# cvg/glue-factory

Measured on AMD Instinct MI355X. Metric: image-pairs/sec (train step) SP+LightGlue N=2048 d=256 L=9, higher is better.
Workload: dtype bf16; 1 GPU; configs[1]: SuperPoint + LightGlue train step -- frozen SuperPoint-open forward on 2x32 synthetic 1024x1024 images resident in HBM (view1 = view0 warped by a sampled homography, SURVEY 8(d)(P); first block and the 64-channel 3x3 blocks as fused HIP kernels, library convolutions + fused HIP tails for the 128/256-channel blocks), homography ground truth (gf_gt_nn), LightGlue fwd + loss + bwd + fused; pairs_per_gpu=32, global_batch=32, keypoints=2048, descriptor_dim=256, layers=9, parallelism=dp1

## Files before the change

glue-factory_amd/csrc/attention.hip:

```cpp
#include "gf_launch.h"
#include "attn_common.h"

using namespace gfattn;

namespace {

bool bad_stride(const int64_t* s, int align) { return s[0] % align || s[1] % align || s[2] % align; }

int attn_params(AttnParams& p, const void* q, const void* k, const void* v, const void* o, const float* lse,
                int B, int H, int Nq, int Nk, int D, const int64_t* qs, const int64_t* ks, const int64_t* vs, const int64_t* os,
                float scale, int dtype, int flags, int known, bool o_f32_if_split) {
    if (D != 64 && D != 32 && D != 128) return GF_ERR_UNSUPPORTED;
    if (flags & ~known) return GF_ERR_UNSUPPORTED;
    if (D != 64 && (flags & GF_ATTN_SPLIT) && dtype != GF_F32) return GF_ERR_UNSUPPORTED;
    if (dtype == GF_F32) flags &= ~GF_ATTN_SPLIT;
    if ((flags & GF_ATTN_SPLIT) && !(kvdma_ok(Nk, ks[1]) && kvdma_ok(Nk, vs[1]))) return GF_ERR_UNSUPPORTED;
    if (B <= 0 || H <= 0 || Nq <= 0 || Nk <= 0) return GF_ERR_SHAPE;
    const int align = gf_vec_elems(dtype);
    if (bad_stride(qs, align) || bad_stride(ks, align) || bad_stride(vs, align) ||
        bad_stride(os, (o_f32_if_split && (flags & GF_ATTN_SPLIT)) ? 4 : align))
        return GF_ERR_ALIGN;
    p = {};
    p.q = q; p.k = k; p.v = v; p.o = const_cast<void*>(o); p.lse = const_cast<float*>(lse);
    p.B = B; p.H = H; p.Nq = Nq; p.Nk = Nk; p.scale = scale;
    host_split_scale(scale, p.p2, p.rr);
    p.flags = flags;
    p.sqb = qs[0]; p.sqn = qs[1]; p.sqh = qs[2];
    p.skb = ks[0]; p.skn = ks[1]; p.skh = ks[2];
    p.svb = vs[0]; p.svn = vs[1]; p.svh = vs[2];
    p.sob = os[0]; p.son = os[1]; p.soh = os[2];
    return 0;
}

bool lds_dma(const AttnParams& p, int dtype, int D) {
    return dtype == GF_BF16 && D == 64 && kvdma_ok(p.Nk, p.skn) && kvdma_ok(p.Nk, p.svn);
}
int launch_fwd(const AttnParams& p, hipStream_t st, int dtype, int D) {
    return lds_dma(p, dtype, D) ? launch_fwd3_bf16(p, st) : launch_fwd_generic(p, st, dtype, D);
}
int launch_bwd(const AttnParams& p, hipStream_t st, int dtype, int D) {
    if (dtype != GF_BF16 || D != 64) return launch_bwd_generic(p, st, dtype, D);
    if (int e = lds_dma(p, dtype, D) ? launch_dq3_bf16(p, st) : launch_dq_generic(p, st, dtype, D)) return e;
    return launch_dkv_bf16(p, st);
}

}

extern "C" int gf_attn_fwd(const void* q, const void* k, const void* v, void* o, float* lse,
                           int B, int H, int Nq, int Nk, int D,
                           const int64_t* q_strides, const int64_t* k_strides,
                           const int64_t* v_strides, const int64_t* o_strides,
                           float scale, int dtype, void* stream) {
    return gf_attn_fwd_ex(q, k, v, o, lse, B, H, Nq, Nk, D, q_strides, k_strides, v_strides, o_strides, scale, dtype, 0, nullptr, stream);
}
extern "C" int gf_attn_fwd_ex(const void* q, const void* k, const void* v, void* o, float* lse,
                              int B, int H, int Nq, int Nk, int D,
                              const int64_t* q_strides, const int64_t* k_strides,
                              const int64_t* v_strides, const int64_t* o_strides,
                              float scale, int dtype, int flags, float* o32, void* stream) {
    AttnParams p;
    if (int e = attn_params(p, q, k, v, o, lse, B, H, Nq, Nk, D, q_strides, k_strides, v_strides, o_strides, scale, dtype,
                            flags, GF_ATTN_SPLIT, false))
        return e;
    p.o32 = (p.flags & GF_ATTN_SPLIT) ? o32 : nullptr;
    return launch_fwd(p, gf_stream(stream), dtype, D);
}

extern "C" int gf_attn_bwd(const void* q, const void* k, const void* v, const void* o,
                           const void* dout, const float* lse, float* delta,
                           void* dq, void* dk, void* dv,
                           int B, int H, int Nq, int Nk, int D,
                           const int64_t* q_strides, const int64_t* k_strides,
                           const int64_t* v_strides, const int64_t* o_strides,
                           const int64_t* do_strides, const int64_t* dq_strides,
                           const int64_t* dk_strides, const int64_t* dv_strides,
                           float scale, int dtype, void* stream) {
    return gf_attn_bwd_acc(q, k, v, o, dout, lse, delta, dq, dk, dv, B, H, Nq, Nk, D, q_strides, k_strides, v_strides, o_strides,
                           do_strides, dq_strides, dk_strides, dv_strides, scale, dtype, 0, stream);
}

extern "C" int gf_attn_bwd_acc(const void* q, const void* k, const void* v, const void* o,
                               const void* dout, const float* lse, float* delta,
                               void* dq, void* dk, void* dv,
                               int B, int H, int Nq, int Nk, int D,
                               const int64_t* q_strides, const int64_t* k_strides,
                               const int64_t* v_strides, const int64_t* o_strides,
                               const int64_t* do_strides, const int64_t* dq_strides,
                               const int64_t* dk_strides, const int64_t* dv_strides,
                               float scale, int dtype, int flags, void* stream) {
    AttnParams p;
    if (int e = attn_params(p, q, k, v, o, lse, B, H, Nq, Nk, D, q_strides, k_strides, v_strides, o_strides, scale, dtype,
                            flags, GF_ATTN_ACC_DQ | GF_ATTN_ACC_DK | GF_ATTN_SPLIT, true))
        return e;
    const int align = gf_vec_elems(dtype);
    if (bad_stride(do_strides, align) || bad_stride(dq_strides, align) || bad_stride(dk_strides, align) || bad_stride(dv_strides, align))
        return GF_ERR_ALIGN;
    p.dout = dout; p.delta = delta; p.dq = dq; p.dk = dk; p.dv = dv;
    p.sdob = do_strides[0]; p.sdon = do_strides[1]; p.sdoh = do_strides[2];
    p.sdqb = dq_strides[0]; p.sdqn = dq_strides[1]; p.sdqh = dq_strides[2];
    p.sdkb = dk_strides[0]; p.sdkn = dk_strides[1]; p.sdkh = dk_strides[2];
    p.sdvb = dv_strides[0]; p.sdvn = dv_strides[1]; p.sdvh = dv_strides[2];
    return launch_bwd(p, gf_stream(stream), dtype, D);
}
```

glue-factory_amd/csrc/attention_fwd3.hip:

```cpp
#include "gf_common.h"
#include "gf_amd.h"
#include "attn_common.h"

namespace gfattn {
namespace {

constexpr float FW3_PS_LIMIT = 65536.f;
#ifndef FW3_ABL
#define FW3_ABL 0
#endif
#ifndef FW3_WPS
#define FW3_WPS 3
#endif

template <bool ZERO>
__device__ __forceinline__ void fw3_scores(f32x16 (&sc)[2], const unsigned (&aR)[4], const bf16x8 (&qf)[4], const f32x16& negm) {
    constexpr int KB = 0;
    u32x4 ka[2][4];
#if FW3_ABL & 2
#pragma unroll
    for (int s = 0; s < 4; ++s) { ka[0][s] = __builtin_bit_cast(u32x4, qf[s]); ka[1][s] = __builtin_bit_cast(u32x4, qf[3 - s]); }
#else
#pragma unroll
    for (int s = 0; s < 4; ++s) ka[0][s] = lds_rd128<KB>(aR[s]);
// ... 110 lines not shown
    GF_FQ_TR(vt0, VB, 0, 0, 0) GF_FQ_TR(vt0, VB, 0, 0, 1) GF_FQ_TR(vt0, VB, 0, 1, 0) GF_FQ_TR(vt0, VB, 0, 1, 1)
    GF_FQ_TR(vt1, VB, 1, 0, 0) GF_FQ_TR(vt1, VB, 1, 0, 1)
    wait_lgkm<4>();
#endif
#if FW3_ABL & 32
#pragma unroll
    for (int db = 0; db < 2; ++db) {
        o[db][0] += (float)p00[0] + (float)p01[0] + (float)p10[0] + (float)p11[0];
        o[db][1] += __builtin_bit_cast(float, vt0[0][db][0][0]) * 1e-30f + __builtin_bit_cast(float, vt1[0][db][0][0]) * 1e-30f;
    }
#else
#pragma unroll
    for (int tt = 0; tt < 2; ++tt) {
#pragma unroll
        for (int db = 0; db < 2; ++db) {
            tie(vt0[tt][db][0]); tie(vt0[tt][db][1]);
            mma16(o[db], as_frag(vt0[tt][db][0], vt0[tt][db][1]), tt ? p01 : p00);
        }
#if !(FW3_ABL & 4)
        if (tt == 0) { GF_FQ_TR(vt1, VB, 1, 1, 0) GF_FQ_TR(vt1, VB, 1, 1, 1) }
#endif
    }
    wait_lgkm<0>();
#pragma unroll
    for (int tt = 0; tt < 2; ++tt)
#pragma unroll
        for (int db = 0; db < 2; ++db) {
            tie(vt1[tt][db][0]); tie(vt1[tt][db][1]);
            mma16(o[db], as_frag(vt1[tt][db][0], vt1[tt][db][1]), tt ? p11 : p10);
        }
#endif
    }
}

template <bool PRE, bool EVEN, bool SPLIT = false>
__global__ __launch_bounds__(256, SPLIT ? 2 : FW3_WPS) void attn_fwd3_bf16_kernel(AttnParams p) {
    extern __shared__ __attribute__((aligned(1024))) char smem[];
    const unsigned lds0 = (unsigned)(size_t)smem;
    const int nqb = (p.Nq + 127) / 128;
    const int total = nqb * p.H * p.B;
    int lb = xcd_remap(blockIdx.x, total);
    const int qb = lb % nqb, h = (lb / nqb) % p.H, b = lb / (nqb * p.H);
    const int lane = threadIdx.x & 63, wave = __builtin_amdgcn_readfirstlane(threadIdx.x >> 6);
    const int l31 = lane & 31, hi = lane >> 5;
    const int qrow = qb * 128 + wave * 32 + l31;
#ifdef FW3_PRIO
    {
        const int pr = (blockIdx.x >> 8) % 3;
        if (pr == 1) __builtin_amdgcn_s_setprio(1); else if (pr == 2) __builtin_amdgcn_s_setprio(2);
    }
#endif

    const bf16_t* qp = reinterpret_cast<const bf16_t*>(p.q) + b * p.sqb + h * p.sqh;
    const bf16_t* kp = reinterpret_cast<const bf16_t*>(p.k) + b * p.skb + h * p.skh;
    const bf16_t* vp = reinterpret_cast<const bf16_t*>(p.v) + b * p.svb + h * p.svh;
    KvDma dma;
    dma.init(kp, vp, p.skn, p.svn, p.Nk, wave, lane);
    const int nt = (p.Nk + 63) / 64;
    if (EVEN) {
        dma.issue_full(0, smem + wave * 1024);
        dma.issue_full(min(1, nt - 1), smem + FQ_STAGE + wave * 1024);
    } else {
        dma.issue(0, smem + wave * 1024);
        if (nt > 1) dma.issue(1, smem + FQ_STAGE + wave * 1024);
    }

    const float p2 = p.p2, rr = PRE ? 1.f : p.rr;
    bf16x8 qf[4];
#pragma unroll
    for (int s = 0; s < 4; ++s) {
        qf[s] = *reinterpret_cast<const bf16x8*>(qp + (int64_t)min(qrow, p.Nq - 1) * p.sqn + 16 * s + 8 * hi);
        if (p2 != 1.f) qf[s] = scale_frag(qf[s], p2);
    }

    f32x16 o[2], negm;
#pragma unroll
    for (int db = 0; db < 2; ++db)
#pragma unroll
        for (int r = 0; r < 16; ++r) o[db][r] = 0.f;
#pragma unroll
    for (int r = 0; r < 16; ++r) negm[r] = -GF_NEG_BIG;
    tie(negm);
    float m = GF_NEG_BIG, lsum = 0.f;
    const FqAddr ad = fq_addresses(lds0, lane);

    unsigned aR[4], aT[4];
#pragma unroll
    for (int i = 0; i < 4; ++i) { aR[i] = ad.aR[i]; aT[i] = ad.aT[i]; }
    int stage = 0;
    if (EVEN) {
        char* const wbase = smem + wave * 1024;
        wait_vm<4>();
        __builtin_amdgcn_s_barrier();
        __builtin_amdgcn_sched_barrier(0);
        dma.issue_full(min(2, nt - 1), wbase + 2 * FQ_STAGE);
        fw3_tile<PRE, SPLIT>(true, 0, p.Nk, aR, aT, qf, o, negm, m, lsum, hi, rr);
#pragma unroll
        for (int i = 0; i < 4; ++i) { aR[i] += FQ_STAGE; aT[i] += FQ_STAGE; }
        stage = 1;
        for (int t = 1; t < nt; ++t) {
            wait_vm<4>();
            __builtin_amdgcn_s_barrier();
            __builtin_amdgcn_sched_barrier(0);
            dma.issue_full(min(t + 2, nt - 1), wbase + (stage == 0 ? 2 : stage - 1) * FQ_STAGE);
            fw3_tile<PRE, SPLIT>(false, t * 64, p.Nk, aR, aT, qf, o, negm, m, lsum, hi, rr);
            const int step = stage == 2 ? -2 * FQ_STAGE : FQ_STAGE;
#pragma unroll
            for (int i = 0; i < 4; ++i) { aR[i] += step; aT[i] += step; }
// ... 62 lines not shown
```

glue-factory_amd/csrc/attn_common.h:

```cpp
#pragma once
#include "gf_launch.h"
#include <cmath>

namespace gfattn {

enum { GF_ATTN_ACC_DQ = 1, GF_ATTN_ACC_DK = 2 };
constexpr int ATTN_PLAIN_STATS = 0x100;

struct AttnParams {
    const void* q; const void* k; const void* v; void* o;
    const void* dout; void* dq; void* dk; void* dv;
    float* lse; float* delta;
    float* o32;
    int B, H, Nq, Nk;
    int64_t sqb, sqn, sqh, skb, skn, skh, svb, svn, svh, sob, son, soh;
    int64_t sdob, sdon, sdoh, sdqb, sdqn, sdqh, sdkb, sdkn, sdkh, sdvb, sdvn, sdvh;
    float scale;
    int flags;
    float p2, rr;
};

template <typename T, int HD> struct Lay {
    static constexpr int VEC = 16 / sizeof(T);
    static constexpr int CPR = HD / VEC;
    static constexpr int LDR = HD + VEC;
    static constexpr int LDT = 64 + 8;
    static constexpr int ROWMAJOR = 64 * LDR;
    static constexpr int TRANSP = HD * LDT;
};

typedef unsigned int u32x4 __attribute__((ext_vector_type(4)));

template <int HD>
__device__ __forceinline__ void add_row(float* rowptr, const f32x16 (&acc)[HD / 32], float mul, int hi) {
#pragma unroll
    for (int db = 0; db < HD / 32; ++db)
#pragma unroll
        for (int g = 0; g < 4; ++g) {
            float* p = rowptr + db * 32 + 8 * g + 4 * hi;
            const f32x4 old = *reinterpret_cast<const f32x4*>(p);
            st4(p, old[0] + acc[db][4 * g] * mul, old[1] + acc[db][4 * g + 1] * mul, old[2] + acc[db][4 * g + 2] * mul,
                old[3] + acc[db][4 * g + 3] * mul);
        }
}
template <int HD>
__device__ __forceinline__ void add_row(bf16_t* rowptr, const f32x16 (&acc)[HD / 32], float mul, int hi) {
#pragma unroll
    for (int db = 0; db < HD / 32; ++db)
#pragma unroll
        for (int g = 0; g < 4; ++g) {
            bf16_t* p = rowptr + db * 32 + 8 * g + 4 * hi;
            const bf16x4 old = *reinterpret_cast<const bf16x4*>(p);
            st4(p, (float)old[0] + acc[db][4 * g] * mul, (float)old[1] + acc[db][4 * g + 1] * mul,
                (float)old[2] + acc[db][4 * g + 2] * mul, (float)old[3] + acc[db][4 * g + 3] * mul);
        }
}

template <typename T, int HD>
__device__ __forceinline__ void store_row(T* rowptr, const f32x16 (&acc)[HD / 32], float mul, int hi) {
#pragma unroll
    for (int db = 0; db < HD / 32; ++db)
#pragma unroll
        for (int g = 0; g < 4; ++g)
            st4(rowptr + db * 32 + 8 * g + 4 * hi, acc[db][4 * g] * mul, acc[db][4 * g + 1] * mul,
                acc[db][4 * g + 2] * mul, acc[db][4 * g + 3] * mul);
}

constexpr int FT_TILE = 8192;
typedef unsigned int u32x2 __attribute__((ext_vector_type(2)));
typedef __attribute__((address_space(3))) void lds_void;
typedef const __attribute__((address_space(1))) void glb_void;
// ... 92 lines not shown
    }
    __device__ __forceinline__ void issue_full(int t, char* dst) const {
        const int sk = t * 64 * skn2, sv = t * 64 * svn2;
        __builtin_amdgcn_raw_ptr_buffer_load_lds(rk, (lds_void*)dst, 16, vk, sk, 0, 0);
        __builtin_amdgcn_raw_ptr_buffer_load_lds(rk, (lds_void*)(dst + 4096), 16, vk, sk + 32 * skn2, 0, 0);
        __builtin_amdgcn_raw_ptr_buffer_load_lds(rv, (lds_void*)(dst + FT_TILE), 16, vv, sv, 0, 0);
        __builtin_amdgcn_raw_ptr_buffer_load_lds(rv, (lds_void*)(dst + FT_TILE + 4096), 16, vv, sv + 32 * svn2, 0, 0);
    }
    __device__ __forceinline__ void issue(int t, char* dst) const {
        const int sk = t * 64 * skn2, sv = t * 64 * svn2;
        if (t * 64 + 64 <= Nk) {
            __builtin_amdgcn_raw_ptr_buffer_load_lds(rk, (lds_void*)dst, 16, vk, sk, 0, 0);
            __builtin_amdgcn_raw_ptr_buffer_load_lds(rk, (lds_void*)(dst + 4096), 16, vk, sk + 32 * skn2, 0, 0);
            __builtin_amdgcn_raw_ptr_buffer_load_lds(rv, (lds_void*)(dst + FT_TILE), 16, vv, sv, 0, 0);
            __builtin_amdgcn_raw_ptr_buffer_load_lds(rv, (lds_void*)(dst + FT_TILE + 4096), 16, vv, sv + 32 * svn2, 0, 0);
        } else {
            int zero;
            asm volatile("s_mov_b32 %0, 0" : "=s"(zero));
            const int rl = Nk - 1 - t * 64, ra = min(r8 + zero, rl), rb = min(r8 + 32 + zero, rl);
            __builtin_amdgcn_raw_ptr_buffer_load_lds(rk, (lds_void*)dst, 16, ra * skn2 + col, sk, 0, 0);
            __builtin_amdgcn_raw_ptr_buffer_load_lds(rk, (lds_void*)(dst + 4096), 16, rb * skn2 + col, sk, 0, 0);
            __builtin_amdgcn_raw_ptr_buffer_load_lds(rv, (lds_void*)(dst + FT_TILE), 16, ra * svn2 + col, sv, 0, 0);
            __builtin_amdgcn_raw_ptr_buffer_load_lds(rv, (lds_void*)(dst + FT_TILE + 4096), 16, rb * svn2 + col, sv, 0, 0);
        }
    }
};
inline bool kvdma_ok(int64_t rows, int64_t ld) { return rows * ld < (1 << 29); }

inline void host_split_scale(float scale, float& p2, float& rr) {
    const double c = (double)scale * 1.4426950408889634074;
    int e;
    double m = std::frexp(c, &e);
    m *= 2.0; e -= 1;
    if (m - 1.0 < 1e-6) m = 1.0;
    if (2.0 - m < 2e-6) { m = 1.0; e += 1; }
    p2 = (float)std::ldexp(1.0, e);
    rr = (float)m;
}
__device__ __forceinline__ bf16x8 scale_frag(bf16x8 v, float p2) {
    bf16x8 r;
#pragma unroll
    for (int e = 0; e < 8; ++e) r[e] = (bf16_t)((float)v[e] * p2);
    return r;
}

template <typename K> int set_lds(K kern, size_t bytes) {
    if (bytes > 48 * 1024) {
        if (int e = gf_allow_lds(kern, bytes)) return e;
    }
    return 0;
}

int launch_fwd3_bf16(const AttnParams& p, hipStream_t st);
int launch_dq3_bf16(const AttnParams& p, hipStream_t st);
int launch_dkv_bf16(const AttnParams& p, hipStream_t st);
int launch_fwd_generic(const AttnParams& p, hipStream_t st, int dtype, int D);
int launch_dq_generic(const AttnParams& p, hipStream_t st, int dtype, int D);
int launch_bwd_generic(const AttnParams& p, hipStream_t st, int dtype, int D);

}
```

glue-factory_amd/ops/__init__.py:

```python
from ._base import BF16, F32, _chk, _dt, _p, _s3, _stream
from ._attention import (ATTN_SPLIT, LN2, SharedGradSum, attention, attention_qkv, attn_bwd_raw, attn_fwd_raw, attn_premul,
                         cross_attention, cross_attention_stacked, self_attention_rotary)
from ._params import (_LP_CACHE, _LP_FLAT, _LP_PTR, _LP_T, _DerivedWeight, _lp, _wt_t, derived_weight, folded_linear,
                      invalidate_precast, precast)
from ._linear import (LIBRARY_GEMMS, GradChain, colsum, gemm, gemm_takes, linear, linear_cat, ln_gelu, rowdot, rowdot2,
                      small_linear)
from ._nll import _SPARSE_SUMS, _known_sums, nll_positive_terms, nll_terms
from ._assignment import (_head_bwd, assign_write, bgemm, dual_lse, dual_lse_stacked, filter_matches, lg_layer_loss,
                          n_pair_loss, nn_filter, rows_argmax, rows_lse, rows_top2, similarity)
from ._sinkhorn import sinkhorn, sinkhorn_schedule
from ._batchnorm import (COLLECTIVES, _BatchNormActSetsSync, _ReplayRunningStats, batch_norm_act, batch_norm_act_sets,
                         replay_running_stats)
from ._lines import (_line_graph_sorted, dense_log_double_softmax, line_aggregate, line_gather, line_graph, line_pair_scores,
                     rows_gather)

XBWD_ENABLED = True

FOLD_ENABLED = True

REPLAY_GATE = None

FORCE_SYNC_BN = False

from ..data._views_ops import filter_views, warp_views
```

glue-factory_amd/ops/_attention.py:

```python
import weakref

import torch

from .. import lib as _lib
from ._base import _chk, _dt, _p, _s3, _stream


ATTN_SPLIT = 4


def attn_fwd_raw(q, k, v, scale, out=None, lse=None, split=False, o32=None):
    _chk(q, k, v)
    B, Nq, H, D = q.shape
    Nk = k.shape[1]
    o = torch.empty((B, Nq, H, D), dtype=q.dtype, device=q.device) if out is None else out
    if lse is None:
        lse = torch.empty((B, H, Nq), dtype=torch.float32, device=q.device)
    split = bool(split) and q.dtype == torch.bfloat16
    assert o32 is None or (o32.dtype == torch.float32 and o32.is_contiguous() and tuple(o32.shape) == (B, Nq, H, D))
    _lib.check(_lib.load().gf_attn_fwd_ex(_p(q), _p(k), _p(v), _p(o), _p(lse), B, H, Nq, Nk, D,
                                          _s3(q), _s3(k), _s3(v), _s3(o), float(scale), _dt(q), ATTN_SPLIT if split else 0,
                                          _p(o32) if split else None, _stream()), "gf_attn_fwd_ex")
    return o, lse


def attn_bwd_raw(q, k, v, o, do, lse, dq, dk, dv, scale, acc_dq=False, acc_dk=False, split=False):
    B, Nq, H, D = q.shape
    split = bool(split) and q.dtype == torch.bfloat16
    assert not split or o.dtype == torch.float32
    Nk = k.shape[1]
    if do.stride(3) != 1:
        do = do.contiguous()
    delta = lse.new_empty((2,) + tuple(lse.shape))
    _lib.check(_lib.load().gf_attn_bwd_acc(_p(q), _p(k), _p(v), _p(o), _p(do), _p(lse), _p(delta),
                                       _p(dq), _p(dk), _p(dv), B, H, Nq, Nk, D,
                                       _s3(q), _s3(k), _s3(v), _s3(o), _s3(do), _s3(dq), _s3(dk),
                                       _s3(dv), float(scale), _dt(q),
                                       int(acc_dq) | 2 * int(acc_dk) | (ATTN_SPLIT if split else 0), _stream()),
               "gf_attn_bwd_acc")


class _Attention(torch.autograd.Function):

    @staticmethod
    def forward(ctx, q, k, v, scale, split=False):
        split = bool(split) and q.dtype == torch.bfloat16
        o32 = torch.empty(q.shape, dtype=torch.float32, device=q.device) if split else None
        o, lse = attn_fwd_raw(q, k, v, scale, split=split, o32=o32)
        ctx.save_for_backward(q, k, v, o32 if split else o, lse)
        ctx.scale, ctx.split = scale, split
        return o

    @staticmethod
    def backward(ctx, do):
        q, k, v, o, lse = ctx.saved_tensors
        dq, dk, dv = torch.empty_like(q), torch.empty_like(k), torch.empty_like(v)
        dq, dk, dv = (t.contiguous() for t in (dq, dk, dv))
        attn_bwd_raw(q, k, v, o, do, lse, dq, dk, dv, ctx.scale, split=ctx.split)
        return dq, dk, dv, None, None


def attention(q, k, v, scale=None, split=False):
    scale = q.shape[-1] ** -0.5 if scale is None else scale
    return _Attention.apply(q, k, v, scale, split)


class _SelfAttentionRotary(torch.autograd.Function):

    @staticmethod
    def forward(ctx, qkv, theta, cs, pre_rotated=False, scale=None, theta_sum=None):
        _chk(qkv, cs)
        ctx.theta_sum = theta_sum
        B, N, three, H, D = qkv.shape
        assert three == 3 and qkv.is_contiguous() and cs.is_contiguous() and cs.dtype == torch.float32
# ... 49 lines not shown
            self.acc, self.got = None, 0
            raise RuntimeError(f"SharedGradSum: the backward visited {got} of {self.expected} consumers of a shared tensor -- "
                               "its gradient is incomplete (differentiate through all layers, or build the model without the shared sum)")

    @classmethod
    def check_all(cls):
        for s_ in list(cls.live or ()):
            s_.check()


LN2 = 0.6931471805599453
def attn_premul(head_dim):
    return head_dim ** -0.5 * 1.4426950408889634


def self_attention_rotary(qkv, theta, cs, pre_rotated=False, scale=None, theta_sum=None):
    if theta_sum is not None and not (torch.is_grad_enabled() and theta.requires_grad):
        theta_sum = None
    return _SelfAttentionRotary.apply(qkv, theta, cs, pre_rotated, scale, theta_sum)


class _CrossAttention(torch.autograd.Function):

    @staticmethod
    def forward(ctx, p0, p1, scale=None):
        D = p0.shape[-1]
        sc = ctx.scale = D ** -0.5 if scale is None else scale
        m0, lse0 = attn_fwd_raw(p0[:, :, 0], p1[:, :, 0], p1[:, :, 1], sc)
        m1, lse1 = attn_fwd_raw(p1[:, :, 0], p0[:, :, 0], p0[:, :, 1], sc)
        ctx.save_for_backward(p0, p1, m0, m1, lse0, lse1)
        return m0, m1

    @staticmethod
    def backward(ctx, dm0, dm1):
        p0, p1, m0, m1, lse0, lse1 = ctx.saved_tensors
        D = p0.shape[-1]
        d0, d1 = torch.empty_like(p0), torch.empty_like(p1)
        attn_bwd_raw(p0[:, :, 0], p1[:, :, 0], p1[:, :, 1], m0, dm0, lse0,
                     d0[:, :, 0], d1[:, :, 0], d1[:, :, 1], ctx.scale)
        attn_bwd_raw(p1[:, :, 0], p0[:, :, 0], p0[:, :, 1], m1, dm1, lse1,
                     d1[:, :, 0], d0[:, :, 0], d0[:, :, 1], ctx.scale, acc_dq=True, acc_dk=True)
        return d0, d1, None


class _CrossAttentionStacked(torch.autograd.Function):

    @staticmethod
    def forward(ctx, p, scale=None):
        B2, N, _, H, D = p.shape
        B = B2 // 2
        sc = ctx.scale = D ** -0.5 if scale is None else scale
        m = torch.empty((B2, N, H, D), dtype=p.dtype, device=p.device)
        lse = torch.empty((B2, H, N), dtype=torch.float32, device=p.device)
        p0, p1 = p[:B], p[B:]
        attn_fwd_raw(p0[:, :, 0], p1[:, :, 0], p1[:, :, 1], sc, out=m[:B], lse=lse[:B])
        attn_fwd_raw(p1[:, :, 0], p0[:, :, 0], p0[:, :, 1], sc, out=m[B:], lse=lse[B:])
        ctx.save_for_backward(p, m, lse)
        return m

    @staticmethod
    def backward(ctx, dm):
        from . import XBWD_ENABLED
        p, m, lse = ctx.saved_tensors
        B2, N, _, H, D = p.shape
        B = B2 // 2
        if not dm.is_contiguous():
            dm = dm.contiguous()
        d = torch.empty_like(p)
        if XBWD_ENABLED and p.dtype == torch.bfloat16 and D == 64 and H <= 4 and N % 64 == 0:
            stat = torch.empty((2, B2, H, N), dtype=torch.float32, device=p.device)
            _lib.check(_lib.load().gf_attn_cross_bwd(_p(p[:, :, 0]), _p(p[:, :, 1]), _p(m), _p(dm), _p(lse), _p(stat),
                                                     _p(d[:, :, 0]), _p(d[:, :, 1]), B2, B, H, N, D,
                                                     _s3(p[:, :, 0]), _s3(p[:, :, 1]), _s3(m), _s3(dm), _s3(d[:, :, 0]),
                                                     _s3(d[:, :, 1]), float(ctx.scale), _dt(p), _stream()), "gf_attn_cross_bwd")
            return d, None
        p0, p1, d0, d1 = p[:B], p[B:], d[:B], d[B:]
        attn_bwd_raw(p0[:, :, 0], p1[:, :, 0], p1[:, :, 1], m[:B], dm[:B], lse[:B],
                     d0[:, :, 0], d1[:, :, 0], d1[:, :, 1], ctx.scale)
        attn_bwd_raw(p1[:, :, 0], p0[:, :, 0], p0[:, :, 1], m[B:], dm[B:], lse[B:],
                     d1[:, :, 0], d0[:, :, 0], d0[:, :, 1], ctx.scale, acc_dq=True, acc_dk=True)
        return d, None


def cross_attention(p0, p1, scale=None):
    return _CrossAttention.apply(p0, p1, scale)


def cross_attention_stacked(p, scale=None):
    return _CrossAttentionStacked.apply(p, scale)


class _AttentionQKV(torch.autograd.Function):

    @staticmethod
    def forward(ctx, qkv, cross, scale=None, split=False):
        B2, N, _, H, D = qkv.shape
        sc = ctx.scale = D ** -0.5 if scale is None else scale
        split = bool(split) and qkv.dtype == torch.bfloat16
        o = torch.empty((B2, N, H, D), dtype=qkv.dtype, device=qkv.device)
        o32 = torch.empty((B2, N, H, D), dtype=torch.float32, device=qkv.device) if split else None
        lse = torch.empty((B2, H, N), dtype=torch.float32, device=qkv.device)
        q, k, v = qkv[:, :, 0], qkv[:, :, 1], qkv[:, :, 2]
        if not cross:
            attn_fwd_raw(q, k, v, sc, out=o, lse=lse, split=split, o32=o32)
        else:
            B = B2 // 2
            attn_fwd_raw(q[:B], k[B:], v[B:], sc, out=o[:B], lse=lse[:B], split=split, o32=None if o32 is None else o32[:B])
            attn_fwd_raw(q[B:], k[:B], v[:B], sc, out=o[B:], lse=lse[B:], split=split, o32=None if o32 is None else o32[B:])
        ctx.save_for_backward(qkv, o32 if split else o, lse)
        ctx.cross, ctx.split = cross, split
        return o

    @staticmethod
    def backward(ctx, do):
        qkv, o, lse = ctx.saved_tensors
        B2, N, _, H, D = qkv.shape
        if not do.is_contiguous():
            do = do.contiguous()
        d = torch.empty_like(qkv)
        q, k, v = qkv[:, :, 0], qkv[:, :, 1], qkv[:, :, 2]
        dq, dk, dv = d[:, :, 0], d[:, :, 1], d[:, :, 2]
        sp = ctx.split
        if not ctx.cross:
            attn_bwd_raw(q, k, v, o, do, lse, dq, dk, dv, ctx.scale, split=sp)
        else:
            B = B2 // 2
            attn_bwd_raw(q[:B], k[B:], v[B:], o[:B], do[:B], lse[:B], dq[:B], dk[B:], dv[B:], ctx.scale, split=sp)
            attn_bwd_raw(q[B:], k[:B], v[:B], o[B:], do[B:], lse[B:], dq[B:], dk[:B], dv[:B], ctx.scale, split=sp)
        return d, None, None, None


def attention_qkv(qkv, cross=False, scale=None, split=False):
    return _AttentionQKV.apply(qkv, cross, scale, split)
```

include/gf_amd.h:

```cpp
#ifndef GF_AMD_H
#define GF_AMD_H

#include <stdint.h>

#ifdef __cplusplus
extern "C" {
#endif

#define GF_DTYPE_F32 0
#define GF_DTYPE_BF16 1

#define GF_ERR_UNSUPPORTED (-1)
#define GF_ERR_SHAPE (-2)
#define GF_ERR_ALIGN (-3)
#define GF_ERR_DTYPE (-4)

#define GF_AMD_ABI_VERSION 20
int gf_abi_version(void);

int gf_attn_fwd(const void* q, const void* k, const void* v, void* o, float* lse,
                int B, int H, int Nq, int Nk, int D,
                const int64_t* q_strides, const int64_t* k_strides,
                const int64_t* v_strides, const int64_t* o_strides,
                float scale, int dtype, void* stream);
#define GF_ATTN_SPLIT 4
int gf_attn_fwd_ex(const void* q, const void* k, const void* v, void* o, float* lse,
                   int B, int H, int Nq, int Nk, int D,
                   const int64_t* q_strides, const int64_t* k_strides,
                   const int64_t* v_strides, const int64_t* o_strides,
                   float scale, int dtype, int flags, float* o32, void* stream);

int gf_attn_cross_bwd(const void* qk, const void* v, const void* o, const void* dout, const float* lse, float* stat,
                      void* dqk, void* dv, int B2, int pair, int H, int N, int D,
                      const int64_t* qk_strides, const int64_t* v_strides, const int64_t* o_strides,
                      const int64_t* do_strides, const int64_t* dqk_strides, const int64_t* dv_strides,
                      float scale, int dtype, void* stream);

int gf_attn_bwd(const void* q, const void* k, const void* v, const void* o,
                const void* dout, const float* lse, float* delta,
                void* dq, void* dk, void* dv,
                int B, int H, int Nq, int Nk, int D,
                const int64_t* q_strides, const int64_t* k_strides,
                const int64_t* v_strides, const int64_t* o_strides,
                const int64_t* do_strides, const int64_t* dq_strides,
                const int64_t* dk_strides, const int64_t* dv_strides,
                float scale, int dtype, void* stream);
int gf_attn_bwd_acc(const void* q, const void* k, const void* v, const void* o,
                    const void* dout, const float* lse, float* delta,
                    void* dq, void* dk, void* dv,
                    int B, int H, int Nq, int Nk, int D,
                    const int64_t* q_strides, const int64_t* k_strides,
                    const int64_t* v_strides, const int64_t* o_strides,
                    const int64_t* do_strides, const int64_t* dq_strides,
                    const int64_t* dk_strides, const int64_t* dv_strides,
                    float scale, int dtype, int flags, void* stream);

int gf_rows_lse(const void* a, const void* b, const float* colbias, float* lse,
                int B, int M, int N, int D, int dtype, void* stream);

int gf_rows_argmax(const void* a, const void* b, const float* colbias, float alpha,
                   float* rowmax, int64_t* rowarg,
                   int B, int M, int N, int D, int dtype, void* stream);

int gf_rows_lse_argmax(const void* a, const void* b, const float* bias_z, const float* bias_n,
                       float alpha, float* lse, float* rowmax, int64_t* rowarg,
                       int B, int M, int N, int D, int dtype, void* stream);

int gf_assign_write(const void* a, const void* b, const float* rowbias, const float* colbias,
                    const float* bin_col, const float* bin_row, float alpha, float corner,
                    float* out, float* expsum, int B, int M, int N, int D, int dtype, void* stream);

int gf_dual_softmax_bwd(const void* a, const void* b, const float* r, const float* c,
                        const float* gr, const float* gc, const float* G, int64_t ldg,
                        float galpha, void* dS, int B, int M, int N, int D, int dtype,
                        void* stream);

int gf_head_bwd(const void* a, const void* b, const float* r, const float* c, const float* gr, const float* gc,
                void* da, void* db, int B, int M, int N, int D, int dtype, void* stream);
// ... 242 lines not shown
```

Measured before the change: 532.0 image-pairs/s.

## Add 256-row forward attention kernel and single-launch partner cross attention

Adds a new bf16 D=64 forward attention kernel in which each wave handles two 32-row query groups. Each K/V tile loaded into LDS is therefore reused across 256 query rows per block, with the softmax of one group interleaved with the MMAs of the other. It is selected by default when Nq and Nk are at least 2048 and split mode is off. Separately, cross attention gains a partner flag that has the kernel offset the K/V batch index by B/2, replacing two half-batch launches with one. The costs are more register pressure (launch bounds of 2 blocks per SM), fewer blocks in the grid, and extra dispatch logic.

```diff
diff --git a/glue-factory_amd/csrc/attention.hip b/glue-factory_amd/csrc/attention.hip
--- a/glue-factory_amd/csrc/attention.hip
+++ b/glue-factory_amd/csrc/attention.hip
@@ -35,8 +35,18 @@
 bool lds_dma(const AttnParams& p, int dtype, int D) {
     return dtype == GF_BF16 && D == 64 && kvdma_ok(p.Nk, p.skn) && kvdma_ok(p.Nk, p.svn);
 }
+constexpr int FWD4_MIN_N = 2048;
 int launch_fwd(const AttnParams& p, hipStream_t st, int dtype, int D) {
-    return lds_dma(p, dtype, D) ? launch_fwd3_bf16(p, st) : launch_fwd_generic(p, st, dtype, D);
+    const int forced = p.flags & (GF_ATTN_GEN3 | GF_ATTN_GEN4);
+    if (!lds_dma(p, dtype, D)) {
+        if (forced || p.kv_shift) return GF_ERR_UNSUPPORTED;
+        return launch_fwd_generic(p, st, dtype, D);
+    }
+    if (forced == (GF_ATTN_GEN3 | GF_ATTN_GEN4)) return GF_ERR_UNSUPPORTED;
+    const bool split = (p.flags & GF_ATTN_SPLIT) != 0;
+    if (split && (forced & GF_ATTN_GEN4)) return GF_ERR_UNSUPPORTED;
+    const bool gen4 = !split && (forced ? forced == GF_ATTN_GEN4 : p.Nq >= FWD4_MIN_N && p.Nk >= FWD4_MIN_N);
+    return gen4 ? launch_fwd4_bf16(p, st) : launch_fwd3_bf16(p, st);
 }
 int launch_bwd(const AttnParams& p, hipStream_t st, int dtype, int D) {
     if (dtype != GF_BF16 || D != 64) return launch_bwd_generic(p, st, dtype, D);
@@ -60,8 +70,12 @@
                               float scale, int dtype, int flags, float* o32, void* stream) {
     AttnParams p;
     if (int e = attn_params(p, q, k, v, o, lse, B, H, Nq, Nk, D, q_strides, k_strides, v_strides, o_strides, scale, dtype,
-                            flags, GF_ATTN_SPLIT, false))
+                            flags, GF_ATTN_SPLIT | GF_ATTN_GEN3 | GF_ATTN_GEN4 | GF_ATTN_PARTNER, false))
         return e;
+    if (flags & GF_ATTN_PARTNER) {
+        if (B % 2 || Nq != Nk) return GF_ERR_SHAPE;
+        p.kv_shift = B / 2;
+    }
     p.o32 = (p.flags & GF_ATTN_SPLIT) ? o32 : nullptr;
     return launch_fwd(p, gf_stream(stream), dtype, D);
 }
diff --git a/glue-factory_amd/csrc/attention_fwd3.hip b/glue-factory_amd/csrc/attention_fwd3.hip
--- a/glue-factory_amd/csrc/attention_fwd3.hip
+++ b/glue-factory_amd/csrc/attention_fwd3.hip
@@ -186,8 +186,9 @@
 #endif
 
     const bf16_t* qp = reinterpret_cast<const bf16_t*>(p.q) + b * p.sqb + h * p.sqh;
-    const bf16_t* kp = reinterpret_cast<const bf16_t*>(p.k) + b * p.skb + h * p.skh;
-    const bf16_t* vp = reinterpret_cast<const bf16_t*>(p.v) + b * p.svb + h * p.svh;
+    const int bk = b + p.kv_shift < p.B ? b + p.kv_shift : b + p.kv_shift - p.B;
+    const bf16_t* kp = reinterpret_cast<const bf16_t*>(p.k) + bk * p.skb + h * p.skh;
+    const bf16_t* vp = reinterpret_cast<const bf16_t*>(p.v) + bk * p.svb + h * p.svh;
     KvDma dma;
     dma.init(kp, vp, p.skn, p.svn, p.Nk, wave, lane);
     const int nt = (p.Nk + 63) / 64;
diff --git a/glue-factory_amd/csrc/attention_fwd4.hip b/glue-factory_amd/csrc/attention_fwd4.hip
--- /dev/null
+++ b/glue-factory_amd/csrc/attention_fwd4.hip
@@ -0,0 +1,400 @@
+#include "gf_common.h"
+#include "gf_amd.h"
+#include "attn_common.h"
+
+namespace gfattn {
+namespace {
+
+constexpr float FW4_PS_LIMIT = 65536.f;
+#ifndef FW4_NST
+#define FW4_NST 3
+#endif
+constexpr int FW4_RING = FW4_NST * FQ_STAGE;
+
+__device__ __forceinline__ unsigned fw4_pack2(float a, float b) {
+    const bf16x2 t = {(bf16_t)a, (bf16_t)b};
+    return __builtin_bit_cast(unsigned, t);
+}
+__device__ __forceinline__ bf16x8 fw4_frag(const unsigned (&w)[4]) {
+    const u32x4 v = {w[0], w[1], w[2], w[3]};
+    return __builtin_bit_cast(bf16x8, v);
+}
+__device__ __forceinline__ void fw4_pack(unsigned (&p)[2][2][4], const f32x16 (&sc)[2]) {
+#pragma unroll
+    for (int kb = 0; kb < 2; ++kb)
+#pragma unroll
+        for (int tt = 0; tt < 2; ++tt)
+#pragma unroll
+            for (int i = 0; i < 4; ++i) p[kb][tt][i] = fw4_pack2(sc[kb][8 * tt + 2 * i], sc[kb][8 * tt + 2 * i + 1]);
+}
+__device__ __forceinline__ void fw4_kreads(u32x4 (&ka)[2][4], const unsigned (&aR)[4]) {
+#pragma unroll
+    for (int s = 0; s < 4; ++s) ka[0][s] = lds_rd128<0>(aR[s]);
+#pragma unroll
+    for (int s = 0; s < 4; ++s) ka[1][s] = lds_rd128<4096>(aR[s]);
+}
+__device__ __forceinline__ void fw4_vreads0(u32x2 (&vt)[2][2][2][2], const unsigned (&aT)[4]) {
+    constexpr int VB = FT_TILE;
+    GF_FQ_TR(vt[0], VB, 0, 0, 0) GF_FQ_TR(vt[0], VB, 0, 0, 1) GF_FQ_TR(vt[0], VB, 0, 1, 0) GF_FQ_TR(vt[0], VB, 0, 1, 1)
+}
+__device__ __forceinline__ void fw4_vreads1(u32x2 (&vt)[2][2][2][2], const unsigned (&aT)[4]) {
+    constexpr int VB = FT_TILE;
+    GF_FQ_TR(vt[1], VB, 1, 0, 0) GF_FQ_TR(vt[1], VB, 1, 0, 1) GF_FQ_TR(vt[1], VB, 1, 1, 0) GF_FQ_TR(vt[1], VB, 1, 1, 1)
+}
+
+template <bool PRE, int G>
+__device__ __forceinline__ void fw4_soft4(f32x16 (&sc)[2], unsigned (&p)[2][2][4], float (&ps)[2], float rr) {
+    constexpr int kb = G >> 2, r0 = 4 * (G & 3);
+#pragma unroll
+    for (int r = r0; r < r0 + 4; ++r) {
+        const float e = fast_exp2(PRE ? sc[kb][r] : sc[kb][r] * rr);
+        sc[kb][r] = e;
+        ps[kb] += e;
+    }
+    p[kb][r0 >> 3][(r0 & 7) >> 1] = fw4_pack2(sc[kb][r0], sc[kb][r0 + 1]);
+    p[kb][r0 >> 3][((r0 & 7) >> 1) + 1] = fw4_pack2(sc[kb][r0 + 2], sc[kb][r0 + 3]);
+    tie(p[kb][r0 >> 3][(r0 & 7) >> 1]); tie(p[kb][r0 >> 3][((r0 & 7) >> 1) + 1]);
+}
+
+template <bool PRE>
+__device__ __forceinline__ void fw4_slow_softmax(f32x16 (&sc)[2], int kv0, int Nk, f32x16 (&o)[2], f32x16& negm, float& m, float& lsum,
+                                                 int hi, float rr) {
+    if (kv0 + 64 > Nk) {
+#pragma unroll
+        for (int kb = 0; kb < 2; ++kb)
+#pragma unroll
+            for (int r = 0; r < 16; ++r)
+                if (kv0 + kb * 32 + crow(r, hi) >= Nk) sc[kb][r] = -INFINITY;
+    }
+    float mx = -INFINITY;
+#pragma unroll
+    for (int kb = 0; kb < 2; ++kb)
+#pragma unroll
+        for (int r = 0; r < 16; ++r) mx = fmaxf(mx, sc[kb][r]);
+    mx = fmaxf(mx, xhalf(mx));
+    const float mnew = fmaxf(m, mx);
+    const float alpha = fast_exp2((m - mnew) * rr);
+    m = mnew;
+    lsum *= alpha;
+#pragma unroll
+    for (int db = 0; db < 2; ++db)
+#pragma unroll
+        for (int r = 0; r < 16; ++r) o[db][r] *= alpha;
+#pragma unroll
+    for (int r = 0; r < 16; ++r) negm[r] = -mnew;
+    tie(negm);
+    const float mr = mnew * rr;
+    float ps = 0.f;
+#pragma unroll
+    for (int kb = 0; kb < 2; ++kb)
+#pragma unroll
+        for (int r = 0; r < 16; ++r) {
+            const float e = fast_exp2(fmaf(sc[kb][r], rr, -mr));
+            sc[kb][r] = e;
+            ps += e;
+        }
+    lsum += ps;
+}
+
+template <bool PRE>
+__device__ __forceinline__ void fw4_slow(f32x16 (&sc)[2], int kv0, int Nk, const unsigned (&aR)[4], const bf16x8 (&qf)[4],
+                                         f32x16 (&o)[2], f32x16& negm, float& m, float& lsum, int hi, float rr) {
+#pragma unroll
+    for (int r = 0; r < 16; ++r) { sc[0][r] = 0.f; sc[1][r] = 0.f; }
+#pragma unroll
+    for (int s = 0; s < 4; ++s) {
+        u32x4 k0 = lds_rd128<0>(aR[s]);
+        u32x4 k1 = lds_rd128<4096>(aR[s]);
+        wait_lgkm<0>();
+        tie(k0); tie(k1);
+        mma16(sc[0], as_frag(k0), qf[s]);
+        mma16(sc[1], as_frag(k1), qf[s]);
+    }
+    fw4_slow_softmax<PRE>(sc, kv0, Nk, o, negm, m, lsum, hi, rr);
+}
+
+template <int I, bool WAIT>
+__device__ __forceinline__ void fw4_pv(f32x16 (&o)[2], u32x2 (&vt)[2][2][2][2], const unsigned (&p)[2][2][4], const unsigned (&aT)[4]) {
+    constexpr int kb = I >> 2, tt = (I >> 1) & 1, db = I & 1;
+    if (WAIT) {
+        wait_lgkm<I == 0 ? 6 : 14 - 2 * I>();
+        tie(vt[kb][tt][db][0]); tie(vt[kb][tt][db][1]);
+    }
+    mma16(o[db], as_frag(vt[kb][tt][db][0], vt[kb][tt][db][1]), fw4_frag(p[kb][tt]));
+    if (WAIT && I == 0) fw4_vreads1(vt, aT);
+}
+
+#define FW4_X4(M) M(0) M(1) M(2) M(3)
+#define FW4_X8(M) M(0) M(1) M(2) M(3) M(4) M(5) M(6) M(7)
+
+template <bool PRE>
+__device__ __forceinline__ void fw4_block_tile(bool force_slow, int kv0, int Nk, const unsigned (&aR)[4], const unsigned (&aT)[4],
+                                               const bf16x8 (&qf)[4], f32x16 (&o)[2], f32x16& negm, float& m, float& lsum, int hi, float rr) {
+    f32x16 sc[2];
+    bool slow = force_slow;
+    if (!slow) {
+#pragma unroll
+        for (int s = 0; s < 4; ++s) {
+            u32x4 k0 = lds_rd128<0>(aR[s]);
+            u32x4 k1 = lds_rd128<4096>(aR[s]);
+            wait_lgkm<0>();
+            tie(k0); tie(k1);
+            if (s == 0) { sc[0] = mma16c(as_frag(k0), qf[0], negm); sc[1] = mma16c(as_frag(k1), qf[0], negm); }
+            else { mma16(sc[0], as_frag(k0), qf[s]); mma16(sc[1], as_frag(k1), qf[s]); }
+        }
+        float ps[2] = {0.f, 0.f};
+#pragma unroll
+        for (int kb = 0; kb < 2; ++kb)
+#pragma unroll
+            for (int r = 0; r < 16; ++r) {
+                const float e = fast_exp2(PRE ? sc[kb][r] : sc[kb][r] * rr);
+                sc[kb][r] = e;
+                ps[kb] += e;
+            }
+        const float pt = ps[0] + ps[1];
+        if (__any(!(pt <= FW4_PS_LIMIT))) slow = true;
+        else lsum += pt;
+    }
+    if (slow) fw4_slow<PRE>(sc, kv0, Nk, aR, qf, o, negm, m, lsum, hi, rr);
+    unsigned p[2][2][4];
+    fw4_pack(p, sc);
+#pragma unroll
+    for (int kb = 0; kb < 2; ++kb) {
+        u32x2 vt[2][2][2][2];
+        if (kb == 0) fw4_vreads0(vt, aT); else fw4_vreads1(vt, aT);
+        wait_lgkm<0>();
+#pragma unroll
+        for (int tt = 0; tt < 2; ++tt)
+#pragma unroll
+            for (int db = 0; db < 2; ++db) {
+                tie(vt[kb][tt][db][0]); tie(vt[kb][tt][db][1]);
+                mma16(o[db], as_frag(vt[kb][tt][db][0], vt[kb][tt][db][1]), fw4_frag(p[kb][tt]));
+            }
+    }
+}
+
+template <int S>
+__device__ __forceinline__ void fw4_sstep(f32x16& sc, const u32x4 (&k)[4], const bf16x8 (&qf)[4], const f32x16& negm) {
+    if (S == 0) sc = mma16c(as_frag(k[0]), qf[0], negm);
+    else mma16(sc, as_frag(k[S]), qf[S]);
+}
+
+template <bool PRE>
+__device__ __forceinline__ int fw4_tile_fast(const unsigned (&aR)[4], const unsigned (&aT)[4], const bf16x8 (&qf)[2][4],
+                                             f32x16 (&o)[2][2], const f32x16 (&negm)[2], float (&lsum)[2], float rr) {
+    u32x4 ka[2][4];
+    u32x2 vt[2][2][2][2];
+    f32x16 sa[2], sb[2];
+    unsigned pa[2][2][4], pb[2][2][4];
+    float psa[2] = {0.f, 0.f}, psb[2] = {0.f, 0.f};
+    fw4_kreads(ka, aR);
+    wait_lgkm<4>();
+#pragma unroll
+    for (int s = 0; s < 4; ++s) tie(ka[0][s]);
+#define FW4_S(S) fw4_sstep<S>(sa[0], ka[0], qf[0], negm[0]);
+    FW4_X4(FW4_S)
+#undef FW4_S
+    __builtin_amdgcn_sched_barrier(0);
+#define FW4_S(S) fw4_sstep<S>(sb[0], ka[0], qf[1], negm[1]); fw4_soft4<PRE, S>(sa, pa, psa, rr); __builtin_amdgcn_sched_barrier(0);
+    FW4_X4(FW4_S)
+#undef FW4_S
+    wait_lgkm<0>();
+#pragma unroll
+    for (int s = 0; s < 4; ++s) tie(ka[1][s]);
+#define FW4_S(S) fw4_sstep<S>(sa[1], ka[1], qf[0], negm[0]); fw4_soft4<PRE, S>(sb, pb, psb, rr); __builtin_amdgcn_sched_barrier(0);
+    FW4_X4(FW4_S)
+#undef FW4_S
+#define FW4_S(S) fw4_sstep<S>(sb[1], ka[1], qf[1], negm[1]); if (S == 3) fw4_vreads0(vt, aT); \
+                 fw4_soft4<PRE, 4 + S>(sa, pa, psa, rr); __builtin_amdgcn_sched_barrier(0);
+    FW4_X4(FW4_S)
+#undef FW4_S
+    const float pta = psa[0] + psa[1];
+    if (__any(!(pta <= FW4_PS_LIMIT))) {
+        wait_lgkm<0>();
+        __builtin_amdgcn_sched_barrier(0);
+        return 1;
+    }
+    lsum[0] += pta;
+    __builtin_amdgcn_sched_barrier(0);
+#define FW4_P(I) fw4_pv<I, true>(o[0], vt, pa, aT); fw4_soft4<PRE, 4 + I>(sb, pb, psb, rr); __builtin_amdgcn_sched_barrier(0);
+    FW4_X4(FW4_P)
+#undef FW4_P
+#define FW4_P(I) fw4_pv<4 + I, true>(o[0], vt, pa, aT);
+    FW4_X4(FW4_P)
+#undef FW4_P
+    const float ptb = psb[0] + psb[1];
+    if (__any(!(ptb <= FW4_PS_LIMIT))) return 2;
+    lsum[1] += ptb;
+    __builtin_amdgcn_sched_barrier(0);
+#define FW4_P(I) fw4_pv<I, false>(o[1], vt, pb, aT);
+    FW4_X8(FW4_P)
+#undef FW4_P
+    return 0;
+}
+
+template <bool PRE>
+__device__ __forceinline__ void fw4_tile_first(int Nk, const unsigned (&aR)[4], const unsigned (&aT)[4], const bf16x8 (&qf)[2][4],
+                                               f32x16 (&o)[2][2], f32x16 (&negm)[2], float (&m)[2], float (&lsum)[2], int hi, float rr) {
+    u32x4 ka[2][4];
+    f32x16 sa[2], sb[2];
+    fw4_kreads(ka, aR);
+#pragma unroll
+    for (int r = 0; r < 16; ++r) { sa[0][r] = 0.f; sa[1][r] = 0.f; sb[0][r] = 0.f; sb[1][r] = 0.f; }
+    wait_lgkm<0>();
+#pragma unroll
+    for (int kb = 0; kb < 2; ++kb)
+#pragma unroll
+        for (int s = 0; s < 4; ++s) tie(ka[kb][s]);
+#pragma unroll
+    for (int s = 0; s < 4; ++s)
+#pragma unroll
+        for (int kb = 0; kb < 2; ++kb) {
+            mma16(sa[kb], as_frag(ka[kb][s]), qf[0][s]);
+            mma16(sb[kb], as_frag(ka[kb][s]), qf[1][s]);
+        }
+    u32x2 vt[2][2][2][2];
+    fw4_vreads0(vt, aT);
+    unsigned pa[2][2][4], pb[2][2][4];
+    fw4_slow_softmax<PRE>(sa, 0, Nk, o[0], negm[0], m[0], lsum[0], hi, rr);
+    fw4_pack(pa, sa);
+    fw4_slow_softmax<PRE>(sb, 0, Nk, o[1], negm[1], m[1], lsum[1], hi, rr);
+    fw4_pack(pb, sb);
+    __builtin_amdgcn_sched_barrier(0);
+#define FW4_P(I) fw4_pv<I, true>(o[0], vt, pa, aT);
+    FW4_X8(FW4_P)
+#undef FW4_P
+#define FW4_P(I) fw4_pv<I, false>(o[1], vt, pb, aT);
+    FW4_X8(FW4_P)
+#undef FW4_P
+}
+
+__device__ __forceinline__ void fw4_advance(unsigned (&aR)[4], unsigned (&aT)[4], int& stage) {
+    const int step = stage == FW4_NST - 1 ? -(FW4_NST - 1) * FQ_STAGE : FQ_STAGE;
+#pragma unroll
+    for (int i = 0; i < 4; ++i) { aR[i] += step; aT[i] += step; }
+    stage = stage == FW4_NST - 1 ? 0 : stage + 1;
+}
+
+template <bool PRE, bool EVEN>
+__global__ __launch_bounds__(256, 2) void attn_fwd4_bf16_kernel(AttnParams p) {
+    extern __shared__ __attribute__((aligned(1024))) char smem[];
+    const unsigned lds0 = (unsigned)(size_t)smem;
+    const int nqb = (p.Nq + 255) / 256;
+    const int total = nqb * p.H * p.B;
+    const int lb = xcd_remap(blockIdx.x, total);
+    const int qb = lb % nqb, h = (lb / nqb) % p.H, b = lb / (nqb * p.H);
+    const int bk = b + p.kv_shift < p.B ? b + p.kv_shift : b + p.kv_shift - p.B;
+    const int lane = threadIdx.x & 63, wave = __builtin_amdgcn_readfirstlane(threadIdx.x >> 6);
+    const int l31 = lane & 31, hi = lane >> 5;
+    const int qrow = qb * 256 + wave * 64 + l31;
+
+    const bf16_t* qp = reinterpret_cast<const bf16_t*>(p.q) + b * p.sqb + h * p.sqh;
+    const bf16_t* kp = reinterpret_cast<const bf16_t*>(p.k) + bk * p.skb + h * p.skh;
+    const bf16_t* vp = reinterpret_cast<const bf16_t*>(p.v) + bk * p.svb + h * p.svh;
+    KvDma dma;
+    dma.init(kp, vp, p.skn, p.svn, p.Nk, wave, lane);
+    const int nt = (p.Nk + 63) / 64;
+    char* const wbase = smem + wave * 1024;
+#pragma unroll
+    for (int i = 0; i < FW4_NST - 1; ++i) {
+        if (EVEN) dma.issue_full(min(i, nt - 1), wbase + i * FQ_STAGE);
+        else if (i < nt) dma.issue(i, wbase + i * FQ_STAGE);
+    }
+
+    const float p2 = p.p2, rr = PRE ? 1.f : p.rr;
+    bf16x8 qf[2][4];
+#pragma unroll
+    for (int j = 0; j < 2; ++j)
+#pragma unroll
+        for (int s = 0; s < 4; ++s) {
+            qf[j][s] = *reinterpret_cast<const bf16x8*>(qp + (int64_t)min(qrow + 32 * j, p.Nq - 1) * p.sqn + 16 * s + 8 * hi);
+            if (p2 != 1.f) qf[j][s] = scale_frag(qf[j][s], p2);
+        }
+
+    f32x16 o[2][2], negm[2];
+    float m[2], lsum[2];
+#pragma unroll
+    for (int j = 0; j < 2; ++j) {
+#pragma unroll
+        for (int db = 0; db < 2; ++db)
+#pragma unroll
+            for (int r = 0; r < 16; ++r) o[j][db][r] = 0.f;
+#pragma unroll
+        for (int r = 0; r < 16; ++r) negm[j][r] = -GF_NEG_BIG;
+        tie(negm[j]);
+        m[j] = GF_NEG_BIG; lsum[j] = 0.f;
+    }
+    const FqAddr ad = fq_addresses(lds0, lane);
+    unsigned aR[4], aT[4];
+#pragma unroll
+    for (int i = 0; i < 4; ++i) { aR[i] = ad.aR[i]; aT[i] = ad.aT[i]; }
+    int stage = 0;
+    constexpr int INFL = 4 * (FW4_NST - 2);
+    const int nhot = EVEN ? nt : p.Nk / 64;
+#define FW4_TOP(t) \
+    if (EVEN || nt - 1 - (t) >= FW4_NST - 2) wait_vm<INFL>(); else wait_vm<0>(); \
+    __builtin_amdgcn_s_barrier(); \
+    __builtin_amdgcn_sched_barrier(0); \
+    if (EVEN) dma.issue_full(min((t) + FW4_NST - 1, nt - 1), wbase + (stage == 0 ? FW4_NST - 1 : stage - 1) * FQ_STAGE); \
+    else if ((t) + FW4_NST - 1 < nt) dma.issue((t) + FW4_NST - 1, wbase + (stage == 0 ? FW4_NST - 1 : stage - 1) * FQ_STAGE);
+    FW4_TOP(0)
+    if (p.Nk >= 64) {
+        fw4_tile_first<PRE>(p.Nk, aR, aT, qf, o, negm, m, lsum, hi, rr);
+    } else {
+        fw4_block_tile<PRE>(true, 0, p.Nk, aR, aT, qf[0], o[0], negm[0], m[0], lsum[0], hi, rr);
+        fw4_block_tile<PRE>(true, 0, p.Nk, aR, aT, qf[1], o[1], negm[1], m[1], lsum[1], hi, rr);
+    }
+    fw4_advance(aR, aT, stage);
+    int t = 1, status = 0;
+    while (true) {
+        for (; t < nhot; ++t) {
+            FW4_TOP(t)
+            status = fw4_tile_fast<PRE>(aR, aT, qf, o, negm, lsum, rr);
+            if (status) break;
+            fw4_advance(aR, aT, stage);
+        }
+        if (t >= nt) break;
+        if (status == 0) { FW4_TOP(t) }
+        const bool force = t * 64 + 64 > p.Nk;
+        if (status != 2) fw4_block_tile<PRE>(force, t * 64, p.Nk, aR, aT, qf[0], o[0], negm[0], m[0], lsum[0], hi, rr);
+        fw4_block_tile<PRE>(force, t * 64, p.Nk, aR, aT, qf[1], o[1], negm[1], m[1], lsum[1], hi, rr);
+        fw4_advance(aR, aT, stage);
+        status = 0;
+        ++t;
+    }
+#undef FW4_TOP
+    wait_vm<0>();
+#pragma unroll
+    for (int j = 0; j < 2; ++j) {
+        const float l = lsum[j] + xhalf(lsum[j]);
+        const int qr = qrow + 32 * j;
+        if (qr < p.Nq) {
+            bf16_t* op = reinterpret_cast<bf16_t*>(p.o) + b * p.sob + h * p.soh + (int64_t)qr * p.son;
+            store_row<bf16_t, 64>(op, o[j], 1.f / l, hi);
+            if (hi == 0) p.lse[((int64_t)b * p.H + h) * p.Nq + qr] = (m[j] * rr + fast_log2(l)) * GF_LN2;
+        }
+    }
+}
+
+}
+
+int launch_fwd4_bf16(const AttnParams& p, hipStream_t st) {
+    const int total = ((p.Nq + 255) / 256) * p.H * p.B;
+    const size_t lds = FW4_RING;
+    void (*const kern[4])(AttnParams) = {attn_fwd4_bf16_kernel<false, false>, attn_fwd4_bf16_kernel<false, true>,
+                                         attn_fwd4_bf16_kernel<true, false>, attn_fwd4_bf16_kernel<true, true>};
+    static unsigned long long attr_set = 0;
+    int dev = 0;
+    (void)hipGetDevice(&dev);
+    if (dev >= 64 || !((attr_set >> dev) & 1ull)) {
+        for (auto k : kern) {
+            if (int e = gf_allow_lds(k, lds)) return e;
+        }
+        if (dev < 64) attr_set |= 1ull << dev;
+    }
+    const bool pre = p.rr == 1.f, even = p.Nk % 64 == 0;
+    kern[(pre ? 2 : 0) + (even ? 1 : 0)]<<<dim3(total), dim3(256), lds, st>>>(p);
+    return gf_launched();
+}
+
+}
diff --git a/glue-factory_amd/csrc/attn_common.h b/glue-factory_amd/csrc/attn_common.h
--- a/glue-factory_amd/csrc/attn_common.h
+++ b/glue-factory_amd/csrc/attn_common.h
@@ -17,6 +17,7 @@
     int64_t sdob, sdon, sdoh, sdqb, sdqn, sdqh, sdkb, sdkn, sdkh, sdvb, sdvn, sdvh;
     float scale;
     int flags;
+    int kv_shift;
     float p2, rr;
 };
 
@@ -215,6 +216,7 @@
 }
 
 int launch_fwd3_bf16(const AttnParams& p, hipStream_t st);
+int launch_fwd4_bf16(const AttnParams& p, hipStream_t st);
 int launch_dq3_bf16(const AttnParams& p, hipStream_t st);
 int launch_dkv_bf16(const AttnParams& p, hipStream_t st);
 int launch_fwd_generic(const AttnParams& p, hipStream_t st, int dtype, int D);
diff --git a/glue-factory_amd/ops/__init__.py b/glue-factory_amd/ops/__init__.py
--- a/glue-factory_amd/ops/__init__.py
+++ b/glue-factory_amd/ops/__init__.py
@@ -1,6 +1,6 @@
 from ._base import BF16, F32, _chk, _dt, _p, _s3, _stream
-from ._attention import (ATTN_SPLIT, LN2, SharedGradSum, attention, attention_qkv, attn_bwd_raw, attn_fwd_raw, attn_premul,
-                         cross_attention, cross_attention_stacked, self_attention_rotary)
+from ._attention import (ATTN_GEN, ATTN_PARTNER, ATTN_SPLIT, LN2, SharedGradSum, attention, attention_qkv, attn_bwd_raw,
+                         attn_fwd_raw, attn_premul, cross_attention, cross_attention_stacked, partner_ok, self_attention_rotary)
 from ._params import (_LP_CACHE, _LP_FLAT, _LP_PTR, _LP_T, _DerivedWeight, _lp, _wt_t, derived_weight, folded_linear,
                       invalidate_precast, precast)
 from ._linear import (LIBRARY_GEMMS, GradChain, colsum, gemm, gemm_takes, linear, linear_cat, ln_gelu, rowdot, rowdot2,
diff --git a/glue-factory_amd/ops/_attention.py b/glue-factory_amd/ops/_attention.py
--- a/glue-factory_amd/ops/_attention.py
+++ b/glue-factory_amd/ops/_attention.py
@@ -7,9 +7,16 @@
 
 
 ATTN_SPLIT = 4
-
-
-def attn_fwd_raw(q, k, v, scale, out=None, lse=None, split=False, o32=None):
+ATTN_GEN = {None: 0, 3: 8, 4: 16}
+ATTN_PARTNER = 32
+
+
+def partner_ok(k, v):
+    return (k.dtype == torch.bfloat16 and k.shape[-1] == 64 and k.shape[0] % 2 == 0
+            and k.shape[1] * k.stride(1) < 1 << 29 and v.shape[1] * v.stride(1) < 1 << 29)
+
+
+def attn_fwd_raw(q, k, v, scale, out=None, lse=None, split=False, o32=None, gen=None, partner=False):
     _chk(q, k, v)
     B, Nq, H, D = q.shape
     Nk = k.shape[1]
@@ -19,7 +26,8 @@
     split = bool(split) and q.dtype == torch.bfloat16
     assert o32 is None or (o32.dtype == torch.float32 and o32.is_contiguous() and tuple(o32.shape) == (B, Nq, H, D))
     _lib.check(_lib.load().gf_attn_fwd_ex(_p(q), _p(k), _p(v), _p(o), _p(lse), B, H, Nq, Nk, D,
-                                          _s3(q), _s3(k), _s3(v), _s3(o), float(scale), _dt(q), ATTN_SPLIT if split else 0,
+                                          _s3(q), _s3(k), _s3(v), _s3(o), float(scale), _dt(q),
+                                          (ATTN_SPLIT if split else 0) | ATTN_GEN[gen] | (ATTN_PARTNER if partner else 0),
                                           _p(o32) if split else None, _stream()), "gf_attn_fwd_ex")
     return o, lse
 
@@ -175,9 +183,12 @@
         sc = ctx.scale = D ** -0.5 if scale is None else scale
         m = torch.empty((B2, N, H, D), dtype=p.dtype, device=p.device)
         lse = torch.empty((B2, H, N), dtype=torch.float32, device=p.device)
-        p0, p1 = p[:B], p[B:]
-        attn_fwd_raw(p0[:, :, 0], p1[:, :, 0], p1[:, :, 1], sc, out=m[:B], lse=lse[:B])
-        attn_fwd_raw(p1[:, :, 0], p0[:, :, 0], p0[:, :, 1], sc, out=m[B:], lse=lse[B:])
+        if partner_ok(p[:, :, 0], p[:, :, 1]):
+            attn_fwd_raw(p[:, :, 0], p[:, :, 0], p[:, :, 1], sc, out=m, lse=lse, partner=True)
+        else:
+            p0, p1 = p[:B], p[B:]
+            attn_fwd_raw(p0[:, :, 0], p1[:, :, 0], p1[:, :, 1], sc, out=m[:B], lse=lse[:B])
+            attn_fwd_raw(p1[:, :, 0], p0[:, :, 0], p0[:, :, 1], sc, out=m[B:], lse=lse[B:])
         ctx.save_for_backward(p, m, lse)
         return m
 
@@ -226,6 +237,8 @@
         q, k, v = qkv[:, :, 0], qkv[:, :, 1], qkv[:, :, 2]
         if not cross:
             attn_fwd_raw(q, k, v, sc, out=o, lse=lse, split=split, o32=o32)
+        elif partner_ok(k, v):
+            attn_fwd_raw(q, k, v, sc, out=o, lse=lse, split=split, o32=o32, partner=True)
         else:
             B = B2 // 2
             attn_fwd_raw(q[:B], k[B:], v[B:], sc, out=o[:B], lse=lse[:B], split=split, o32=None if o32 is None else o32[:B])
diff --git a/include/gf_amd.h b/include/gf_amd.h
--- a/include/gf_amd.h
+++ b/include/gf_amd.h
@@ -24,6 +24,9 @@
                 const int64_t* v_strides, const int64_t* o_strides,
                 float scale, int dtype, void* stream);
 #define GF_ATTN_SPLIT 4
+#define GF_ATTN_GEN3 8
+#define GF_ATTN_GEN4 16
+#define GF_ATTN_PARTNER 32
 int gf_attn_fwd_ex(const void* q, const void* k, const void* v, void* o, float* lse,
                    int B, int H, int Nq, int Nk, int D,
                    const int64_t* q_strides, const int64_t* k_strides,
```

Result: no change. 536.0 image-pairs/s, median of 6 (+0.7%).
